# Tencent/PocketFlow

Measured on AMD Instinct MI355X. Metric: images/sec ResNet-50 INT8 quant-aware fine-tune (whole job; per GPU = value / n_gpus), higher is better.
Workload: dtype bf16

## Files before the change

pocketflow_amd/csrc/pf_api.hip:

```cpp
#include "pf_common.h"

extern "C" int pf_version(void) { return 100; }

extern "C" const char* pf_error_string(int err) {
  if (err == 0) return "ok";
  return hipGetErrorString((hipError_t)err);
}

#include <stdlib.h>
#include <stdio.h>
static PfTuning g_tuning;
static bool g_tuning_loaded = false;

static int env_int(const char* name, int dflt) {
  const char* e = getenv(name);
  return (e == nullptr || *e == 0) ? dflt : atoi(e);
}

static void tuning_load() {
  PfTuning t;
  t.conv_bn = env_int("PF_CONV_BN", 0);
  t.conv_igemm = env_int("PF_CONV_IGEMM", 1);
  t.conv_igemm_pro = env_int("PF_CONV_IGEMM_PRO", 1);
  t.conv_stream = env_int("PF_CONV_STREAM", 1);
  t.conv_stream_maxsplit = env_int("PF_CONV_STREAM_MAXSPLIT", 2);
  t.igemm_pro3 = env_int("PF_IGEMM_PRO3", 1);
  t.igemm_tile_bm = t.igemm_tile_bn = 0;
  const char* e = getenv("PF_IGEMM_TILE");
  if (e != nullptr) {
    int bm = 0, bn = 0;
    if (sscanf(e, "%dx%d", &bm, &bn) == 2) { t.igemm_tile_bm = bm; t.igemm_tile_bn = bn; }
  }
  t.pool3s2 = env_int("PF_POOL3S2", 1);
  t.wrw_tr = env_int("PF_WRW_TR", 0);
  t.wrw2 = env_int("PF_WRW2", 1);
  t.wrw2_target = env_int("PF_WRW2_TARGET", 0);
  t.splitk = env_int("PF_IGEMM_SPLITK", 1);
  t.wrw2_tk256 = env_int("PF_WRW2_TK256", 1);
  t.conv3x3_c64 = env_int("PF_CONV3X3_C64", 1);
  g_tuning = t;
  g_tuning_loaded = true;
}

const PfTuning& pf_tuning() {
  if (!g_tuning_loaded) tuning_load();
  return g_tuning;
}

extern "C" int pf_tuning_reload(void) { tuning_load(); return 0; }

#include <map>
#include <mutex>
#include <utility>
int pf_require_lds(const void* fn, size_t lds) {
  static std::mutex mu;
  static std::map<std::pair<int, const void*>, size_t> done;
  int dev = 0;
  hipError_t e = hipGetDevice(&dev);
  if (e != hipSuccess) return (int)e;
  std::lock_guard<std::mutex> lock(mu);
  size_t& have = done[std::make_pair(dev, fn)];
  if (lds > have) {
    e = hipFuncSetAttribute(fn, hipFuncAttributeMaxDynamicSharedMemorySize, (int)lds);
    if (e != hipSuccess) return (int)e;
    have = lds;
  }
  return 0;
}
```

pocketflow_amd/csrc/pf_common.h:

```cpp
#pragma once
#include <hip/hip_runtime.h>
#include <stdint.h>
#include "../../include/pocketflow_hip.h"

#define PF_WAVE 64
#define PF_THREADS 256
#define PF_MAX_GRID 2048

#define PF_LAUNCH_CHECK()                         \
  do {                                            \
    hipError_t e__ = hipGetLastError();           \
    if (e__ != hipSuccess) return (int)e__;       \
  } while (0)

typedef uint16_t bf16_t;

int pf_require_lds(const void* fn, size_t lds);

struct PfTuning {
  int conv_bn;
  int conv_igemm, conv_igemm_pro;
  int conv_stream;
  int conv_stream_maxsplit;
  int igemm_pro3;
  int igemm_tile_bm, igemm_tile_bn;
  int pool3s2;
  int wrw_tr, wrw2, wrw2_target;
  int wrw2_tk256;
  int splitk;
  int conv3x3_c64;
};
const PfTuning& pf_tuning();

__device__ __forceinline__ float bf16_to_f32(bf16_t h) {
  return __uint_as_float(((uint32_t)h) << 16);
}
__device__ __forceinline__ bf16_t f32_to_bf16(float f) {
  uint32_t u = __float_as_uint(f);
  if ((u & 0x7FFFFFFFu) > 0x7F800000u) return (bf16_t)((u >> 16) | 0x0040u);
  u += 0x7FFFu + ((u >> 16) & 1u);
  return (bf16_t)(u >> 16);
}

template <typename T> struct VecTraits;
template <> struct VecTraits<float> { static constexpr int N = 4; };
template <> struct VecTraits<bf16_t> { static constexpr int N = 8; };

template <typename T>
__device__ __forceinline__ void load_vec(const T* __restrict__ p, float* out);
template <>
__device__ __forceinline__ void load_vec<float>(const float* __restrict__ p, float* out) {
  float4 v = *reinterpret_cast<const float4*>(p);
  out[0] = v.x; out[1] = v.y; out[2] = v.z; out[3] = v.w;
}
template <>
__device__ __forceinline__ void load_vec<bf16_t>(const bf16_t* __restrict__ p, float* out) {
  uint4 v = *reinterpret_cast<const uint4*>(p);
  out[0] = __uint_as_float(v.x << 16); out[1] = __uint_as_float(v.x & 0xFFFF0000u);
  out[2] = __uint_as_float(v.y << 16); out[3] = __uint_as_float(v.y & 0xFFFF0000u);
  out[4] = __uint_as_float(v.z << 16); out[5] = __uint_as_float(v.z & 0xFFFF0000u);
  out[6] = __uint_as_float(v.w << 16); out[7] = __uint_as_float(v.w & 0xFFFF0000u);
}
template <typename T>
__device__ __forceinline__ void store_vec(T* __restrict__ p, const float* in);
template <>
__device__ __forceinline__ void store_vec<float>(float* __restrict__ p, const float* in) {
  *reinterpret_cast<float4*>(p) = make_float4(in[0], in[1], in[2], in[3]);
}
template <>
__device__ __forceinline__ void store_vec<bf16_t>(bf16_t* __restrict__ p, const float* in) {
  uint4 v;
  v.x = (uint32_t)f32_to_bf16(in[0]) | ((uint32_t)f32_to_bf16(in[1]) << 16);
  v.y = (uint32_t)f32_to_bf16(in[2]) | ((uint32_t)f32_to_bf16(in[3]) << 16);
  v.z = (uint32_t)f32_to_bf16(in[4]) | ((uint32_t)f32_to_bf16(in[5]) << 16);
  v.w = (uint32_t)f32_to_bf16(in[6]) | ((uint32_t)f32_to_bf16(in[7]) << 16);
  *reinterpret_cast<uint4*>(p) = v;
}
template <typename T> __device__ __forceinline__ void load8(const T* __restrict__ p, float* out);
template <> __device__ __forceinline__ void load8<float>(const float* __restrict__ p, float* out) {
  load_vec<float>(p, out); load_vec<float>(p + 4, out + 4);
}
template <> __device__ __forceinline__ void load8<bf16_t>(const bf16_t* __restrict__ p, float* out) {
  load_vec<bf16_t>(p, out);
}
template <typename T> __device__ __forceinline__ void store8(T* __restrict__ p, const float* in);
template <> __device__ __forceinline__ void store8<float>(float* __restrict__ p, const float* in) {
  store_vec<float>(p, in); store_vec<float>(p + 4, in + 4);
}
template <> __device__ __forceinline__ void store8<bf16_t>(bf16_t* __restrict__ p, const float* in) {
  store_vec<bf16_t>(p, in);
}
__host__ __device__ __forceinline__ bool pf_aligned16(const void* p) {
  return (((uintptr_t)p) & 15) == 0;
}
template <typename T> __device__ __forceinline__ float load_one(const T* p);
template <> __device__ __forceinline__ float load_one<float>(const float* p) { return *p; }
template <> __device__ __forceinline__ float load_one<bf16_t>(const bf16_t* p) { return bf16_to_f32(*p); }
template <typename T> __device__ __forceinline__ void store_one(T* p, float v);
template <> __device__ __forceinline__ void store_one<float>(float* p, float v) { *p = v; }
template <> __device__ __forceinline__ void store_one<bf16_t>(bf16_t* p, float v) { *p = f32_to_bf16(v); }

__device__ __forceinline__ uint32_t enc_f32(float f) {
  uint32_t u = __float_as_uint(f);
  return (u & 0x80000000u) ? ~u : (u | 0x80000000u);
}
__device__ __forceinline__ float dec_f32(uint32_t e) {
  uint32_t u = (e & 0x80000000u) ? (e & 0x7FFFFFFFu) : ~e;
  return __uint_as_float(u);
}
__device__ __forceinline__ void slot_alpha_beta(const uint32_t* slot, float& alpha, float& beta) {
  const uint2 sv = *reinterpret_cast<const uint2*>(slot);
// ... 71 lines not shown
```

pocketflow_amd/csrc/pf_conv.hip:

```cpp
#include "pf_conv_common.h"

template <int BN_T, bool PRO, bool BWD, bool MAP>
__global__ __launch_bounds__(PF_THREADS, 2) void k_conv1x1_fwd(const ConvArgs a) {
  constexpr int WM = (BN_T == 128) ? 64 : 32;
  constexpr int JM = WM / 16;
  constexpr int CS_LD = BN_T + 8;
  constexpr int VPR = BN_T / 8;
  constexpr int RPP = PF_THREADS / VPR;
  constexpr int NBV = BN_T * 8 / PF_THREADS;
  constexpr int A_EL = CV_BM * CV_LDK, B_EL = BN_T * CV_LDK;
  constexpr int C_EL = CV_BM * CS_LD;
  constexpr int RED_FL = 4 * RPP * BN_T;
  constexpr int SM_BYTES_AB = (A_EL + B_EL) * 2;
  constexpr int SM_BYTES = SM_BYTES_AB > RED_FL * 4 ? (SM_BYTES_AB > C_EL * 2 ? SM_BYTES_AB : C_EL * 2)
                                                    : RED_FL * 4;
  constexpr int SS_BYTES = PRO ? 2 * CV_MAXK * 4 : 0;
  __shared__ __attribute__((aligned(16))) unsigned char smem[SM_BYTES + SS_BYTES];
  float* ssl = reinterpret_cast<float*>(smem + SM_BYTES);
  __shared__ float bpl[BWD ? 4 * BN_T : 4];
  bf16_t* As = reinterpret_cast<bf16_t*>(smem);
  bf16_t* Bs = As + A_EL;
  bf16_t* Cs = reinterpret_cast<bf16_t*>(smem);
  float* red = reinterpret_cast<float*>(smem);

// ... 476 lines not shown
      if (vq[i]) v = *reinterpret_cast<const uint4*>(a.X + map_row(a, m) * a.K + k);
      rq[i] = v;
    }
  };
  auto sstore = [&]() {
#pragma unroll
    for (int i = 0; i < 4; ++i) {
      const int p = tid + i * PF_THREADS;
      st_transposed(Ds, (p & 15) * 8, p >> 4, rd[i]);
    }
#pragma unroll
    for (int i = 0; i < 2; ++i) {
      const int p = tid + i * PF_THREADS;
      uint4 v = rq[i];
      if (PRO) v = vq[i] ? pro_apply(pro, v) : make_uint4(0, 0, 0, 0);
      st_transposed(Qs, (p & 7) * 8, p >> 3, v);
    }
  };

  if (mbeg < mend) gload(mbeg);
  for (int mb = mbeg; mb < mend; mb += WR_BM) {
    sstore();
    __syncthreads();
    if (mb + WR_BM < mend) gload(mb + WR_BM);
#pragma unroll
    for (int kk = 0; kk < WR_BM / 32; ++kk) {
      bf16x8 df[2], qf[4];
      const int mg = kk * 4 + fm;
#pragma unroll
      for (int i = 0; i < 2; ++i) {
        const int c = wave * 32 + i * 16 + frow;
        df[i] = *reinterpret_cast<const bf16x8*>(Ds + c * WR_LDM + ((mg ^ ((c >> 3) & 7)) << 3));
      }
#pragma unroll
      for (int j = 0; j < 4; ++j) {
        const int c = j * 16 + frow;
        qf[j] = *reinterpret_cast<const bf16x8*>(Qs + c * WR_LDM + ((mg ^ ((c >> 3) & 7)) << 3));
      }
#pragma unroll
      for (int i = 0; i < 2; ++i)
#pragma unroll
        for (int j = 0; j < 4; ++j)
          acc[i][j] = __builtin_amdgcn_mfma_f32_16x16x32_bf16(df[i], qf[j], acc[i][j], 0, 0, 0);
    }
    __syncthreads();
  }
  float* out = a.partial + (int64_t)split * a.N * a.K;
#pragma unroll
  for (int i = 0; i < 2; ++i)
#pragma unroll
    for (int j = 0; j < 4; ++j) {
      const int k = k0 + j * 16 + (lane & 15);
#pragma unroll
      for (int r = 0; r < 4; ++r) {
        const int n = n0 + wave * 32 + i * 16 + (lane >> 4) * 4 + r;
        if (n < a.N && k < a.K) out[(int64_t)n * a.K + k] = acc[i][j][r];
      }
    }
}

template <typename TO>
__global__ __launch_bounds__(PF_THREADS) void k_wrw_reduce(const float* __restrict__ partial, int splits,
                                                           int64_t n, TO* __restrict__ out, int64_t out_stride) {
  __shared__ float l[4][64];
  const int e_l = threadIdx.x & 63, sg = threadIdx.x >> 6;
  const int64_t e = (int64_t)blockIdx.x * 64 + e_l;
  const int per = (splits + gridDim.y - 1) / gridDim.y;
  const int s0 = blockIdx.y * per, s1 = (s0 + per < splits) ? (s0 + per) : splits;
  float acc = 0.f;
  if (e < n)
    for (int s = s0 + sg; s < s1; s += 4) acc += partial[(int64_t)s * n + e];
  l[sg][e_l] = acc;
  __syncthreads();
  if (sg == 0 && e < n) store_one<TO>(out + (int64_t)blockIdx.y * out_stride + e, (l[0][e_l] + l[1][e_l]) + (l[2][e_l] + l[3][e_l]));
}

WrwPlan pf_wrw_plan(int M, int N, int C, int taps, bool entry_1x1, int64_t x_rows, int window_imgs);
int pf_wrw2_launch(const void* dY, const void* X, float* slabs, const float* scale_shift, int act, const uint32_t* slot,
                   int bits, int M, int N, int C, int th, int tw, int H, int Wd, int Ho, int Wo, int stride, int pad_h,
                   int pad_w, int S, int64_t x_rows, hipStream_t st);
int pf_wrw_tr_launch(const void* dY, const void* X, float* slabs, const float* scale_shift, int act,
                     const uint32_t* slot, int bits, int M, int N, int C, int th, int tw, int H, int Wd, int Ho, int Wo,
                     int stride, int pad_h, int pad_w, int S, hipStream_t st);

int pf_wrw_reduce(float* workspace, int S, int64_t n, void* dW, int dw_dtype, hipStream_t st) {
  const int gx = (int)((n + 63) / 64);
  int ry = 1;
  while (ry < 32 && gx * ry < 1024 && ry * 8 <= S) ry *= 2;
  float* stage = workspace + (int64_t)S * n;
  if (ry > 1) {
    k_wrw_reduce<float><<<dim3(gx, ry), PF_THREADS, 0, st>>>(workspace, S, n, stage, n);
    if (dw_dtype == PF_F32) k_wrw_reduce<float><<<dim3(gx, 1), PF_THREADS, 0, st>>>(stage, ry, n, (float*)dW, 0);
    else if (dw_dtype == PF_BF16) k_wrw_reduce<bf16_t><<<dim3(gx, 1), PF_THREADS, 0, st>>>(stage, ry, n, (bf16_t*)dW, 0);
    else return (int)hipErrorInvalidValue;
  } else {
    if (dw_dtype == PF_F32) k_wrw_reduce<float><<<dim3(gx, 1), PF_THREADS, 0, st>>>(workspace, S, n, (float*)dW, 0);
    else if (dw_dtype == PF_BF16) k_wrw_reduce<bf16_t><<<dim3(gx, 1), PF_THREADS, 0, st>>>(workspace, S, n, (bf16_t*)dW, 0);
    else return (int)hipErrorInvalidValue;
  }
  PF_LAUNCH_CHECK();
  return 0;
}

int pf_wrw_scatter_splits(int M, int N, int K) {
  const int tiles = ((N + WR_TN - 1) / WR_TN) * ((K + WR_TK - 1) / WR_TK);
  int S = (768 + tiles - 1) / tiles;
  const int maxS = (M + 4 * WR_BM - 1) / (4 * WR_BM);
  if (S > maxS) S = maxS;
  if (S < 1) S = 1;
  int rows = (M + S - 1) / S;
  rows = ((rows + WR_BM - 1) / WR_BM) * WR_BM;
  return (M + rows - 1) / rows;
}

extern "C" int pf_conv1x1_wrw_splits(int M, int N, int K) { return pf_wrw_plan(M, N, K, 1, true, 0, 0).S; }

extern "C" int pf_conv1x1_wrw(const void* dY, const void* X, void* dW, int dw_dtype, float* workspace,
                              const float* scale_shift, int act, const uint32_t* slot, int bits, int M, int N,
                              int K, int Ho, int Wo, int H, int Wd, int stride, void* stream) {
  if (M <= 0 || N <= 0 || K <= 0 || (K % 8) || (N % 8) || ((int64_t)N * K) % 4) return (int)hipErrorInvalidValue;
  if (!pf_aligned16(dY) || !pf_aligned16(X) || !pf_aligned16(workspace) || !pf_aligned16(dW))
    return (int)hipErrorInvalidValue;
  if (slot != nullptr && (bits < 1 || bits > 32 || scale_shift == nullptr)) return (int)hipErrorInvalidValue;
  if (stride < 1) stride = 1;
  hipStream_t st = (hipStream_t)stream;
  if (stride > 1 && (Ho <= 0 || Wo <= 0 || H <= 0 || Wd <= 0)) return (int)hipErrorInvalidValue;
  const int64_t x_rows = (stride > 1) ? (int64_t)(M / (Ho * Wo)) * H * Wd : (int64_t)M;
  const WrwPlan p = pf_wrw_plan(M, N, K, 1, true, x_rows, 0);
  int r = 0;
  if (p.kernel == WRW_SHARED) {
    r = pf_wrw2_launch(dY, X, workspace, scale_shift, act, slot, bits, M, N, K, 1, 1, H, Wd, Ho, Wo, stride, 0, 0, p.S, x_rows, st);
  } else if (p.kernel == WRW_WAVE) {
    r = pf_wrw_tr_launch(dY, X, workspace, scale_shift, act, slot, bits, M, N, K, 1, 1, H, Wd, Ho, Wo, stride, 0, 0, p.S, st);
  } else {
    ConvArgs a = conv_args(X, dY, nullptr, M, N, K);
    conv_args_prologue(a, scale_shift, act, slot, bits);
    conv_args_rowmap(a, Ho, Wo, H, Wd, stride, 0);
    a.partial = workspace;
    a.tiles_n = (N + WR_TN - 1) / WR_TN;
    const int tiles_k = (K + WR_TK - 1) / WR_TK;
    int rows = (M + p.S - 1) / p.S;
    rows = ((rows + WR_BM - 1) / WR_BM) * WR_BM;
    a.rows_per_split = rows;
    dim3 grid(a.tiles_n * tiles_k, p.S);
    if (scale_shift != nullptr) k_conv1x1_wrw<true><<<grid, PF_THREADS, 0, st>>>(a);
    else k_conv1x1_wrw<false><<<grid, PF_THREADS, 0, st>>>(a);
    PF_LAUNCH_CHECK();
  }
  if (r != 0) return r;
  return pf_wrw_reduce(workspace, p.S, (int64_t)N * K, dW, dw_dtype, st);
}
```

pocketflow_amd/csrc/pf_wrw.hip:

```cpp
#include "pf_conv_common.h"
#include <stdlib.h>

#define LDS_PTR(p) ((__attribute__((address_space(3))) void*)(p))
typedef short v4s __attribute__((ext_vector_type(4)));
typedef short v8s __attribute__((ext_vector_type(8)));

__device__ __attribute__((aligned(16))) const uint32_t pf_wrw_zero_page[64] = {0};

struct WrwArgs {
  const bf16_t* dY;
  const bf16_t* X;
  float* slabs;
  const float* ss;
  const uint32_t* slot;
  float kq, act_lo, act_hi;
  int M, N, C;
  int th, tw, H, Wd, Ho, Wo, stride, pad_h, pad_w;
  int tiles_n, tiles, rows_per_split;
};

template <int N> __device__ __forceinline__ void wrw_wait_vm() { asm volatile("s_waitcnt vmcnt(%0)" ::"n"(N) : "memory"); }

template <int BN, bool PRO, bool MAP>
__global__ __launch_bounds__(256) void k_wrw_tr(const WrwArgs a) {
  constexpr int NB = BN / 16;
  constexpr int NS = 3;
  constexpr int DY_BYTES = 4 * NB * 256, X_BYTES = 4 * 4 * 256, STAGE = DY_BYTES + X_BYTES;
  constexpr int LPS = NB + 4;
  constexpr int NBLK = NB * 4;
  extern __shared__ __attribute__((aligned(16))) unsigned char smem[];
  const int tid = threadIdx.x, lane = tid & 63;
  const int wave = __builtin_amdgcn_readfirstlane(tid >> 6);
  const int l15 = lane & 15, q = lane >> 4;
  unsigned char* ring = smem + wave * (NS * STAGE);
  const bf16_t* zero = reinterpret_cast<const bf16_t*>(pf_wrw_zero_page);

  const int nwg = gridDim.x;
  int wg = blockIdx.x;
  {
    const int xcd = wg & 7, idx = wg >> 3;
    const int qq = nwg >> 3, r = nwg & 7;
    wg = (xcd < r ? xcd * (qq + 1) : r * (qq + 1) + (xcd - r) * qq) + idx;
  }
  const int tile = wg % a.tiles, split = wg / a.tiles;
  const int tn = tile % a.tiles_n, tk = tile / a.tiles_n;
  const int n0 = tn * BN;
  const int cch = a.C >> 6;
  const int tap = tk / cch, c0 = (tk - tap * cch) * 64;
  const int tap_r = tap / a.tw, tap_s = tap - tap_r * a.tw;
  const int ktot = a.th * a.tw * a.C;
  const int mbeg = split * a.rows_per_split;
  const int mend = (mbeg + a.rows_per_split < a.M) ? (mbeg + a.rows_per_split) : a.M;
  const int nsteps = (mend > mbeg) ? (mend - mbeg + 31) / 32 : 0;
  const int my_steps = (nsteps > wave) ? (nsteps - wave + 3) / 4 : 0;

  float psc[4], psh[4];
  Pro pro;
  pro_init(pro, a.act_lo, a.act_hi, a.kq, PRO ? a.slot : nullptr);
  if (PRO) {
#pragma unroll
    for (int j = 0; j < 4; ++j) {
      psc[j] = pro_fold_scale(pro, a.ss[c0 + j * 16 + l15]);
      psh[j] = pro_fold_shift(pro, a.ss[a.C + c0 + j * 16 + l15]);
    }
  }

  const int sb = lane >> 4, srow = (lane & 15) >> 1, sch = lane & 1;
  const int hw_o = a.Ho * a.Wo;
  auto stage = [&](int step, int buf) {
    unsigned char* dst = ring + buf * STAGE;
    const int mb = mbeg + step * 32;
#pragma unroll
    for (int pg = 0; pg < 4; ++pg) {
      const int m = mb + pg * 8 + srow;
      const bool ok = m < mend;
#pragma unroll
      for (int g4 = 0; g4 < NB / 4; ++g4) {
        const int n = n0 + (g4 * 4 + sb) * 16 + sch * 8;
        const bf16_t* src = (ok && n < a.N) ? (a.dY + (int64_t)m * a.N + n) : (zero + sch * 8);
        __builtin_amdgcn_global_load_lds(src, LDS_PTR(dst + (pg * NB + g4 * 4) * 256), 16, 0, 0);
      }
      bool okx = ok;
      int64_t row = m;
      if (MAP && ok) {
// ... 162 lines not shown
#define PF_W_MAKE_RSRC(p, bytes) __builtin_amdgcn_make_buffer_rsrc((void*)(p), (short)0, (int)(bytes), 0x00020000)
#define PF_W_BUFFER_LOAD_LDS16(rs, lds, voff) __builtin_amdgcn_raw_ptr_buffer_load_lds(rs, LDS_PTR(lds), 16, voff, 0, 0, 0)
#else
typedef int pf_wrsrc_t;
#define PF_W_MAKE_RSRC(p, bytes) 0
#define PF_W_BUFFER_LOAD_LDS16(rs, lds, voff) ((void)(rs), (void)(lds), (void)(voff))
#endif

#ifndef PF_W2_ABLATE
#define PF_W2_ABLATE 0
#endif
#ifdef PF_W2_TIMING
#define PF_W2_STAMP(k) do { if (blockIdx.x == (unsigned)tm_blk && t >= 4 && t < 12 && lane == 0) \
    tm_out[(t - 4) * 8 + (k)] = (uint32_t)__builtin_readcyclecounter(); } while (0)
#else
#define PF_W2_STAMP(k) do { } while (0)
#endif

__device__ __forceinline__ bf16x8 tr_join(const v4s& lo, const v4s& hi) {
  v8s x8;
  x8[0] = lo[0]; x8[1] = lo[1]; x8[2] = lo[2]; x8[3] = lo[3];
  x8[4] = hi[0]; x8[5] = hi[1]; x8[6] = hi[2]; x8[7] = hi[3];
  return *reinterpret_cast<const bf16x8*>(&x8);
}
template <int HI>
__device__ __forceinline__ void tr_read_frags(uint32_t p, bf16x8 (&f)[4]) {
  v4s l0, l1, l2, l3, h0, h1, h2, h3;
  asm volatile("ds_read_b64_tr_b16 %0, %8\n\tds_read_b64_tr_b16 %4, %8 offset:%9\n\t"
               "ds_read_b64_tr_b16 %1, %8 offset:256\n\tds_read_b64_tr_b16 %5, %8 offset:%10\n\t"
               "ds_read_b64_tr_b16 %2, %8 offset:512\n\tds_read_b64_tr_b16 %6, %8 offset:%11\n\t"
               "ds_read_b64_tr_b16 %3, %8 offset:768\n\tds_read_b64_tr_b16 %7, %8 offset:%12\n\t"
               "s_waitcnt lgkmcnt(0)"
               : "=&v"(l0), "=&v"(l1), "=&v"(l2), "=&v"(l3), "=&v"(h0), "=&v"(h1), "=&v"(h2), "=&v"(h3)
               : "v"(p), "n"(HI), "n"(HI + 256), "n"(HI + 512), "n"(HI + 768)
               : "memory");
  f[0] = tr_join(l0, h0); f[1] = tr_join(l1, h1); f[2] = tr_join(l2, h2); f[3] = tr_join(l3, h3);
}
template <int HI>
__device__ __forceinline__ void tr_read_frags(uint32_t p, bf16x8 (&f)[2]) {
  v4s l0, l1, h0, h1;
  asm volatile("ds_read_b64_tr_b16 %0, %4\n\tds_read_b64_tr_b16 %2, %4 offset:%5\n\t"
               "ds_read_b64_tr_b16 %1, %4 offset:256\n\tds_read_b64_tr_b16 %3, %4 offset:%6\n\t"
               "s_waitcnt lgkmcnt(0)"
               : "=&v"(l0), "=&v"(l1), "=&v"(h0), "=&v"(h1)
               : "v"(p), "n"(HI), "n"(HI + 256)
               : "memory");
  f[0] = tr_join(l0, h0); f[1] = tr_join(l1, h1);
}

template <int HIX, int HID>
__device__ __forceinline__ void tr_read_frags2(uint32_t px, uint32_t pd, bf16x8 (&xf)[4], bf16x8 (&df)[4]) {
  v4s a0, a1, a2, a3, b0, b1, b2, b3, c0, c1, c2, c3, d0, d1, d2, d3;
  asm volatile("ds_read_b64_tr_b16 %0, %16\n\tds_read_b64_tr_b16 %4, %16 offset:%18\n\t"
               "ds_read_b64_tr_b16 %1, %16 offset:256\n\tds_read_b64_tr_b16 %5, %16 offset:%19\n\t"
               "ds_read_b64_tr_b16 %2, %16 offset:512\n\tds_read_b64_tr_b16 %6, %16 offset:%20\n\t"
               "ds_read_b64_tr_b16 %3, %16 offset:768\n\tds_read_b64_tr_b16 %7, %16 offset:%21\n\t"
               "ds_read_b64_tr_b16 %8, %17\n\tds_read_b64_tr_b16 %12, %17 offset:%22\n\t"
               "ds_read_b64_tr_b16 %9, %17 offset:256\n\tds_read_b64_tr_b16 %13, %17 offset:%23\n\t"
               "ds_read_b64_tr_b16 %10, %17 offset:512\n\tds_read_b64_tr_b16 %14, %17 offset:%24\n\t"
               "ds_read_b64_tr_b16 %11, %17 offset:768\n\tds_read_b64_tr_b16 %15, %17 offset:%25\n\t"
               "s_waitcnt lgkmcnt(0)"
               : "=&v"(a0), "=&v"(a1), "=&v"(a2), "=&v"(a3), "=&v"(b0), "=&v"(b1), "=&v"(b2), "=&v"(b3),
                 "=&v"(c0), "=&v"(c1), "=&v"(c2), "=&v"(c3), "=&v"(d0), "=&v"(d1), "=&v"(d2), "=&v"(d3)
               : "v"(px), "v"(pd), "n"(HIX), "n"(HIX + 256), "n"(HIX + 512), "n"(HIX + 768), "n"(HID), "n"(HID + 256), "n"(HID + 512),
                 "n"(HID + 768)
               : "memory");
  xf[0] = tr_join(a0, b0); xf[1] = tr_join(a1, b1); xf[2] = tr_join(a2, b2); xf[3] = tr_join(a3, b3);
  df[0] = tr_join(c0, d0); df[1] = tr_join(c1, d1); df[2] = tr_join(c2, d2); df[3] = tr_join(c3, d3);
}

struct Wrw2Args {
  const bf16_t* dY;
  const bf16_t* X;
  float* slabs;
  const float* ss;
  const uint32_t* slot;
  float kq, act_lo, act_hi;
  uint32_t dy_bytes, x_bytes;
  int M, N, C;
  int th, tw, H, Wd, Ho, Wo, stride, pad_h, pad_w;
  int tiles_n, tiles, rows_per_split;
};

template <int TN, int TK, int WTN, int WTK, bool PRO, int MAPM>
__global__ __launch_bounds__(64 * (TN / WTN) * (TK / WTK)) void k_wrw2(const Wrw2Args a) {
  constexpr int WN = TN / WTN, WK = TK / WTK, NWAVE = WN * WK;
  constexpr int NI = WTN / 16, NJ = WTK / 16;
  constexpr int NBN = TN / 16, NBK = TK / 16;
  constexpr int DY_BYTES = 4 * NBN * 256, X_BYTES = 4 * NBK * 256, STAGE = DY_BYTES + X_BYTES;
  constexpr int IDY = 4 * (TN / 64), IX = 4 * (TK / 64);
  static_assert(IDY % NWAVE == 0 || IDY < NWAVE, "dY instructions must split evenly over the wavefronts (slot kinds are static)");
  constexpr int KDY = (IDY + NWAVE - 1) / NWAVE;
  constexpr int XS = (IX + NWAVE - 1) / NWAVE;
  extern __shared__ __attribute__((aligned(16))) unsigned char smem[];
  const int tid = threadIdx.x, lane = tid & 63;
  const int wave = __builtin_amdgcn_readfirstlane(tid >> 6);
  const int l15 = lane & 15, q = lane >> 4;
  const int wn = wave / WK, wk = wave % WK;

  const int nwg = gridDim.x;
  int wg = blockIdx.x;
  {
    const int xcd = wg & 7, idx = wg >> 3;
    const int qq = nwg >> 3, r = nwg & 7;
    wg = (xcd < r ? xcd * (qq + 1) : r * (qq + 1) + (xcd - r) * qq) + idx;
  }
  const int tile = wg % a.tiles, split = wg / a.tiles;
  const int tn = tile % a.tiles_n, tk = tile / a.tiles_n;
  const int n0 = tn * TN;
  const int kt = a.C / TK;
  const int tap = tk / kt, c0 = (tk - tap * kt) * TK;
  const int tap_r = tap / a.tw, tap_s = tap - tap_r * a.tw;
  const int ktot = a.th * a.tw * a.C;
  const int mbeg = split * a.rows_per_split;
  const int mend = (mbeg + a.rows_per_split < a.M) ? (mbeg + a.rows_per_split) : a.M;
  const int nsteps = (mend > mbeg) ? (mend - mbeg + 31) / 32 : 0;

  const pf_wrsrc_t rsY = PF_W_MAKE_RSRC(a.dY, (uint32_t)mend * (uint32_t)a.N * 2u);
  const pf_wrsrc_t rsX = PF_W_MAKE_RSRC(a.X, (MAPM == 0) ? (uint32_t)mend * (uint32_t)a.C * 2u : a.x_bytes);
  constexpr uint32_t OOB = 0x80000000u;
  const int sb = lane >> 4, srow = (lane & 15) >> 1, sch = lane & 1;
  const int hw_o = a.Ho * a.Wo;

  float psc[XS][8], psh[XS][8];
  Pro pro;
  pro_init(pro, a.act_lo, a.act_hi, a.kq, PRO ? a.slot : nullptr);
  if (PRO) {
#pragma unroll
    for (int x = 0; x < XS; ++x) {
      const int xi = wave + x * NWAVE;
      if (xi < IX) {
        const int g4 = xi % (TK / 64);
        const int c = c0 + (g4 * 4 + sb) * 16 + sch * 8;
#pragma unroll
        for (int j = 0; j < 8; ++j) { psc[x][j] = pro_fold_scale(pro, a.ss[c + j]); psh[x][j] = pro_fold_shift(pro, a.ss[a.C + c + j]); }
      }
    }
  }

  uint32_t yoff[KDY], xoff[XS];
  const uint32_t ystep = 32u * (uint32_t)a.N * 2u, xstep = 32u * (uint32_t)a.C * 2u;
#pragma unroll
  for (int k = 0; k < KDY; ++k) {
    const int id = (wave + k * NWAVE) % IDY;
    const int pg = id / (TN / 64), g4 = id % (TN / 64);
    const int n = n0 + (g4 * 4 + sb) * 16 + sch * 8;
    yoff[k] = (n < a.N && wave + k * NWAVE < IDY) ? (uint32_t)((mbeg + pg * 8 + srow) * a.N + n) * 2u : OOB;
  }
  int px_img[XS], px_ho[XS], px_wo[XS];
  const int adv_q = 32 / a.Wo, adv_r = 32 - adv_q * a.Wo;
  const int tap_dr = tap_r - a.pad_h, tap_ds = tap_s - a.pad_w;
#pragma unroll
  for (int x = 0; x < XS; ++x) {
    const int xi = (wave + x * NWAVE) % IX;
    const int pg = xi / (TK / 64), g4 = xi % (TK / 64);
    const int m = mbeg + pg * 8 + srow;
    const int cofs = c0 + (g4 * 4 + sb) * 16 + sch * 8;
    px_img[x] = 0; px_ho[x] = 0; px_wo[x] = 0;
    if (MAPM != 0) {
      const int img = m / hw_o, rem = m - img * hw_o;
      px_img[x] = img; px_ho[x] = rem / a.Wo; px_wo[x] = rem - px_ho[x] * a.Wo;
    }
    const int row0 = (MAPM == 1) ? m + tap_dr * a.Wd + tap_ds : m;
    xoff[x] = (uint32_t)(row0 * a.C + cofs) * 2u;
  }
  auto stage = [&](int step, int buf) {
    unsigned char* dst = smem + buf * STAGE;
// ... 36 lines not shown
      }
      if (!own) voff = OOB;
      unsigned char* xdst = own ? dst + DY_BYTES + (pg * NBK + g4 * 4) * 256 : smem + 3 * STAGE;
      if (!(PF_W2_ABLATE & 2)) PF_W_BUFFER_LOAD_LDS16(rsX, xdst, voff);
    }
  };
  auto transform = [&](int buf) {
    unsigned char* dst = smem + buf * STAGE;
#pragma unroll
    for (int x = 0; x < XS; ++x) {
      const int xi = wave + x * NWAVE;
      if (xi < IX) {
        const int pg = xi / (TK / 64), g4 = xi % (TK / 64);
#pragma unroll
        for (int j = 0; j < 8; ++j) { pro.sc[j] = psc[x][j]; pro.sh[j] = psh[x][j]; }
        const uint32_t p = lds_addr(dst + DY_BYTES + (pg * NBK + g4 * 4) * 256 + lane * 16);
        lds_write_b128(p, pro_apply(pro, lds_read_b128(p)));
      }
    }
  };

  f32x4 acc[NI][NJ];
#pragma unroll
  for (int i = 0; i < NI; ++i)
#pragma unroll
    for (int j = 0; j < NJ; ++j) acc[i][j] = (f32x4){0.f, 0.f, 0.f, 0.f};
  const int tr_off = (q & 1) * 128 + (l15 >> 2) * 32 + (l15 & 3) * 8;
  const int pg_lo = q >> 1;

  constexpr int NSTG = 3, LPS = KDY + XS;
  if (nsteps > 0) stage(0, 0);
  if (nsteps > 1) { stage(1, 1); wrw_wait_vm<LPS>(); } else wrw_wait_vm<0>();
  if (PRO && nsteps > 0) transform(0);
  asm volatile("s_waitcnt lgkmcnt(0)" ::: "memory");
  __builtin_amdgcn_s_barrier();
  int buf = 0, ibuf = 2;
#ifdef PF_W2_TIMING
  const int tm_blk = gridDim.x / 2;
  uint32_t* tm_out = reinterpret_cast<uint32_t*>(a.slabs) + wave * 64;
#endif
  for (int t = 0; t < nsteps; ++t) {
    const bool more2 = t + 2 < nsteps;
    PF_W2_STAMP(0);
    if (more2) { stage(t + 2, ibuf); ibuf = (ibuf + 1 == NSTG) ? 0 : ibuf + 1; }
    PF_W2_STAMP(1);
    const unsigned char* sbase = smem + buf * STAGE;
    buf = (buf + 1 == NSTG) ? 0 : buf + 1;
    if (!(PF_W2_ABLATE & 1)) {
      bf16x8 xf[NJ], df[NI];
      if constexpr (NI == 4 && NJ == 4) {
        tr_read_frags2<2 * NBK * 256, 2 * NBN * 256>(lds_addr(sbase + DY_BYTES + (pg_lo * NBK + wk * NJ) * 256 + tr_off),
                                                     lds_addr(sbase + (pg_lo * NBN + wn * NI) * 256 + tr_off), xf, df);
      } else
      {
      tr_read_frags<2 * NBK * 256>(lds_addr(sbase + DY_BYTES + (pg_lo * NBK + wk * NJ) * 256 + tr_off), xf);
      tr_read_frags<2 * NBN * 256>(lds_addr(sbase + (pg_lo * NBN + wn * NI) * 256 + tr_off), df);
      }
      PF_W2_STAMP(2);
#pragma unroll
      for (int i = 0; i < NI; ++i)
#pragma unroll
        for (int j = 0; j < NJ; ++j)
          acc[i][j] = __builtin_amdgcn_mfma_f32_16x16x32_bf16(df[i], xf[j], acc[i][j], 0, 0, 0);
    }
    __builtin_amdgcn_sched_barrier(0);
    PF_W2_STAMP(3);
    if (t + 1 < nsteps) {
      if (more2) wrw_wait_vm<LPS>(); else wrw_wait_vm<0>();
      PF_W2_STAMP(4);
      if (PRO) transform(buf);
    }
    asm volatile("s_waitcnt lgkmcnt(0)" ::: "memory");
    PF_W2_STAMP(5);
    __builtin_amdgcn_s_barrier();
    __builtin_amdgcn_sched_barrier(0);
    PF_W2_STAMP(6);
  }
#ifdef PF_W2_TIMING
  return;
#endif

  float* out = a.slabs + (int64_t)split * a.N * ktot;
  const int kcol = tap * a.C + c0 + wk * WTK;
#pragma unroll
  for (int i = 0; i < NI; ++i)
#pragma unroll
    for (int j = 0; j < NJ; ++j) {
      const int k = kcol + j * 16 + l15;
      const int n = n0 + wn * WTN + i * 16 + q * 4;
#pragma unroll
      for (int r = 0; r < 4; ++r)
        if (n + r < a.N && (!(PF_W2_ABLATE & 4) || acc[i][j][r] == 12345.678f)) out[(int64_t)(n + r) * ktot + k] = acc[i][j][r];
    }
}

struct Wrw2Cfg { int tn, tk; };
static Wrw2Cfg wrw2_pick(int N, int C) {
  const int tn = (N % 256 == 0) ? 256 : ((N % 128 == 0) ? 128 : 64);
  int tk = (C % 128 == 0) ? 128 : 64;
  if (tn <= 128 && C % 256 == 0 && pf_tuning().wrw2_tk256 != 0) tk = 256;
  if (tn == 128 && tk == 64) return Wrw2Cfg{64, 64};
  return Wrw2Cfg{tn, tk};
}

static bool wrw2_fits(int M, int N, int C, int64_t x_rows) {
  return (int64_t)M * N < ((int64_t)1 << 30) && x_rows * C < ((int64_t)1 << 30);
}

int pf_wrw2_splits(int M, int N, int C, int taps) {
  if (pf_tuning().wrw2 == 0) return 0;
  if ((C % 64) || (N % 64) || M < 2048 || !wrw2_fits(M, N, C, 0)) return 0;
  const Wrw2Cfg c = wrw2_pick(N, C);
  const int tiles = (N / c.tn) * (taps * C / c.tk);
  const int forced = pf_tuning().wrw2_target;
  const int target = (forced > 0) ? forced : (taps == 1 ? 256 : 384);
  int S = (target + tiles - 1) / tiles;
  const int maxS = (M + 255) / 256;
  if (S > maxS) S = maxS;
  if (S < 1) S = 1;
  int rows = (M + S - 1) / S;
  rows = ((rows + 31) / 32) * 32;
  return (M + rows - 1) / rows;
}

template <int TN, int TK, int WTN, int WTK, bool PRO, int MAPM>
static int wrw2_launch_t(const Wrw2Args& a, int grid, hipStream_t st) {
  const size_t lds = 3 * (size_t)(4 * (TN / 16) * 256 + 4 * (TK / 16) * 256) + 1024;
  if (int e = pf_require_lds(reinterpret_cast<const void*>(&k_wrw2<TN, TK, WTN, WTK, PRO, MAPM>), lds)) return e;
  k_wrw2<TN, TK, WTN, WTK, PRO, MAPM><<<grid, 64 * (TN / WTN) * (TK / WTK), lds, st>>>(a);
  PF_LAUNCH_CHECK();
  return 0;
}

int pf_wrw2_launch(const void* dY, const void* X, float* slabs, const float* scale_shift, int act, const uint32_t* slot,
                   int bits, int M, int N, int C, int th, int tw, int H, int Wd, int Ho, int Wo, int stride, int pad_h,
                   int pad_w, int S, int64_t x_rows, hipStream_t st) {
  if (S <= 0 || !wrw2_fits(M, N, C, x_rows)) return (int)hipErrorInvalidValue;
  Wrw2Args a;
  a.dY = (const bf16_t*)dY; a.X = (const bf16_t*)X; a.slabs = slabs; a.ss = scale_shift; a.slot = slot;
  a.kq = uq_k_of_bits(slot ? bits : 8);
  pf_act_window(act, &a.act_lo, &a.act_hi);
  a.dy_bytes = (uint32_t)((int64_t)M * N * 2);
  a.x_bytes = (uint32_t)(x_rows * C * 2);
  a.M = M; a.N = N; a.C = C; a.th = th; a.tw = tw; a.H = H; a.Wd = Wd; a.Ho = Ho; a.Wo = Wo;
  a.stride = stride; a.pad_h = pad_h; a.pad_w = pad_w;
  const Wrw2Cfg c = wrw2_pick(N, C);
  a.tiles_n = N / c.tn;
  a.tiles = a.tiles_n * (th * tw * C / c.tk);
  int rows = (M + S - 1) / S;
  rows = ((rows + 31) / 32) * 32;
  a.rows_per_split = rows;
  const int grid = a.tiles * S;
  const bool pro = scale_shift != nullptr;
  int mapm = 0;
  if (stride != 1 || th * tw > 1) mapm = (stride == 1 && Ho == H && Wo == Wd && 32 / Wo + 1 <= Ho) ? 1 : 2;
  if (pro && th * tw > 1) return (int)hipErrorInvalidValue;
  if (pro && mapm == 1) mapm = 2;
#define PF_W2(TNV, TKV, WTNV, WTKV)                                                                           \
  do {                                                                                                        \
    if (pro) return mapm ? wrw2_launch_t<TNV, TKV, WTNV, WTKV, true, 2>(a, grid, st)                           \
                         : wrw2_launch_t<TNV, TKV, WTNV, WTKV, true, 0>(a, grid, st);                          \
    if (mapm == 1) return wrw2_launch_t<TNV, TKV, WTNV, WTKV, false, 1>(a, grid, st);                          \
    return mapm ? wrw2_launch_t<TNV, TKV, WTNV, WTKV, false, 2>(a, grid, st)                                   \
                : wrw2_launch_t<TNV, TKV, WTNV, WTKV, false, 0>(a, grid, st);                                  \
  } while (0)
  if (c.tn == 128 && c.tk == 256) PF_W2(128, 256, 64, 64);
  if (c.tn == 64 && c.tk == 256) PF_W2(64, 256, 32, 64);
  if (c.tn == 256 && c.tk == 128) PF_W2(256, 128, 64, 64);
  if (c.tn == 128 && c.tk == 128) PF_W2(128, 128, 64, 64);
  if (c.tn == 256 && c.tk == 64) PF_W2(256, 64, 64, 32);
  if (c.tn == 64 && c.tk == 128) PF_W2(64, 128, 32, 64);
  PF_W2(64, 64, 32, 32);
#undef PF_W2
}

int pf_wrw_reduce(float* workspace, int S, int64_t n, void* dW, int dw_dtype, hipStream_t st);

bool pf_wrw3x3_c64_geom(int H, int Wd, int C, int N, int th, int tw, int stride, int pad_h, int pad_w, int Ho, int Wo);
bool pf_wrw3x3_c64_fits(int imgs);
int pf_wrw3x3_c64_splits(int imgs);
int pf_wrw3x3_c64_launch(const void* dY, const void* X, float* slabs, int imgs, hipStream_t st);
int pf_wrw_scatter_splits(int M, int N, int K);

WrwPlan pf_wrw_plan(int M, int N, int C, int taps, bool entry_1x1, int64_t x_rows, int window_imgs) {
  if (window_imgs > 0 && pf_wrw3x3_c64_fits(window_imgs)) return WrwPlan{WRW_WINDOW, pf_wrw3x3_c64_splits(window_imgs)};
  const int s2 = pf_wrw2_splits(M, N, C, taps);
  if (s2 > 0) return WrwPlan{wrw2_fits(M, N, C, x_rows) ? WRW_SHARED : WRW_WAVE, s2};
  const int s1 = (!entry_1x1 || pf_tuning().wrw_tr != 0) ? wrw_tr_splits(M, N, C, taps) : 0;
  if (s1 > 0) return WrwPlan{WRW_WAVE, s1};
  if (entry_1x1) return WrwPlan{WRW_SCATTER, pf_wrw_scatter_splits(M, N, C)};
  return WrwPlan{WRW_NONE, 0};
}

extern "C" int pf_conv2d_wrw_splits(int M, int N, int C, int taps) {
  const int s = pf_wrw_plan(M, N, C, taps, false, 0, 0).S;
  if (pf_tuning().conv3x3_c64 != 0 && taps == 9 && N == 64 && C == 64 && M % (56 * 56) == 0) {
    const int s3 = pf_wrw_plan(M, N, C, taps, false, 0, M / (56 * 56)).S;
    return s3 > s ? s3 : s;
  }
  return s;
}

extern "C" int pf_conv2d_wrw(const void* dY, const void* X, void* dW, int dw_dtype, float* workspace, int imgs, int H,
                             int Wd, int C, int N, int th, int tw, int stride, int pad_h, int pad_w, int Ho, int Wo,
                             void* stream) {
  if (imgs <= 0 || H <= 0 || Wd <= 0 || Ho <= 0 || Wo <= 0 || th < 1 || tw < 1 || stride < 1) return (int)hipErrorInvalidValue;
  if (!pf_aligned16(dY) || !pf_aligned16(X) || !pf_aligned16(dW) || !pf_aligned16(workspace)) return (int)hipErrorInvalidValue;
  const int M = imgs * Ho * Wo;
  hipStream_t st = (hipStream_t)stream;
  const bool window = pf_wrw3x3_c64_geom(H, Wd, C, N, th, tw, stride, pad_h, pad_w, Ho, Wo);
  const WrwPlan p = pf_wrw_plan(M, N, C, th * tw, false, (int64_t)imgs * H * Wd, window ? imgs : 0);
  int r = (int)hipErrorInvalidValue;
  if (p.kernel == WRW_WINDOW) r = pf_wrw3x3_c64_launch(dY, X, workspace, imgs, st);
  if (p.kernel == WRW_SHARED)
    r = pf_wrw2_launch(dY, X, workspace, nullptr, PF_ACT_NONE, nullptr, 8, M, N, C, th, tw, H, Wd, Ho, Wo, stride, pad_h, pad_w, p.S,
                       (int64_t)imgs * H * Wd, st);
  if (p.kernel == WRW_WAVE)
    r = pf_wrw_tr_launch(dY, X, workspace, nullptr, PF_ACT_NONE, nullptr, 8, M, N, C, th, tw, H, Wd, Ho, Wo, stride, pad_h, pad_w, p.S, st);
  if (r != 0) return r;
  return pf_wrw_reduce(workspace, p.S, (int64_t)N * th * tw * C, dW, dw_dtype, st);
}
```

Measured before the change: 11410.

## Store wrw2 partials in MFMA fragment layout and add matching fragment-aware reduce

The weight-gradient wrw2 kernel now writes each accumulator fragment as one contiguous float4 per lane in a 16x16-blocked layout instead of a row-major scatter, which makes the partial-slab stores coalesced. A new two-stage reduce kernel sums the split slabs in that blocked layout, optionally staging through extra workspace, and transposes back to row-major dW in the final pass. This is on by default through PF_WRW2_FRAG. It adds constraints that N and ktot be multiples of 16, needs extra workspace for the staging pass, and may add a launch.

```diff
diff --git a/pocketflow_amd/csrc/pf_api.hip b/pocketflow_amd/csrc/pf_api.hip
--- a/pocketflow_amd/csrc/pf_api.hip
+++ b/pocketflow_amd/csrc/pf_api.hip
@@ -37,6 +37,7 @@
   t.wrw2_target = env_int("PF_WRW2_TARGET", 0);
   t.splitk = env_int("PF_IGEMM_SPLITK", 1);
   t.wrw2_tk256 = env_int("PF_WRW2_TK256", 1);
+  t.wrw2_frag = env_int("PF_WRW2_FRAG", 1);
   t.conv3x3_c64 = env_int("PF_CONV3X3_C64", 1);
   g_tuning = t;
   g_tuning_loaded = true;
diff --git a/pocketflow_amd/csrc/pf_common.h b/pocketflow_amd/csrc/pf_common.h
--- a/pocketflow_amd/csrc/pf_common.h
+++ b/pocketflow_amd/csrc/pf_common.h
@@ -27,6 +27,7 @@
   int pool3s2;
   int wrw_tr, wrw2, wrw2_target;
   int wrw2_tk256;
+  int wrw2_frag;
   int splitk;
   int conv3x3_c64;
 };
diff --git a/pocketflow_amd/csrc/pf_conv.hip b/pocketflow_amd/csrc/pf_conv.hip
--- a/pocketflow_amd/csrc/pf_conv.hip
+++ b/pocketflow_amd/csrc/pf_conv.hip
@@ -582,6 +582,7 @@
 int pf_wrw_tr_launch(const void* dY, const void* X, float* slabs, const float* scale_shift, int act,
                      const uint32_t* slot, int bits, int M, int N, int C, int th, int tw, int H, int Wd, int Ho, int Wo,
                      int stride, int pad_h, int pad_w, int S, hipStream_t st);
+int pf_wrw2_reduce(float* workspace, int S, int N, int ktot, void* dW, int dw_dtype, hipStream_t st);
 
 int pf_wrw_reduce(float* workspace, int S, int64_t n, void* dW, int dw_dtype, hipStream_t st) {
   const int gx = (int)((n + 63) / 64);
@@ -648,5 +649,6 @@
     PF_LAUNCH_CHECK();
   }
   if (r != 0) return r;
+  if (p.kernel == WRW_SHARED) return pf_wrw2_reduce(workspace, p.S, N, K, dW, dw_dtype, st);
   return pf_wrw_reduce(workspace, p.S, (int64_t)N * K, dW, dw_dtype, st);
 }
diff --git a/pocketflow_amd/csrc/pf_wrw.hip b/pocketflow_amd/csrc/pf_wrw.hip
--- a/pocketflow_amd/csrc/pf_wrw.hip
+++ b/pocketflow_amd/csrc/pf_wrw.hip
@@ -1,5 +1,6 @@
 #include "pf_conv_common.h"
 #include <stdlib.h>
+#include <type_traits>
 
 #define LDS_PTR(p) ((__attribute__((address_space(3))) void*)(p))
 typedef short v4s __attribute__((ext_vector_type(4)));
@@ -328,7 +329,7 @@
   int tiles_n, tiles, rows_per_split;
 };
 
-template <int TN, int TK, int WTN, int WTK, bool PRO, int MAPM>
+template <int TN, int TK, int WTN, int WTK, bool PRO, int MAPM, bool FRAG>
 __global__ __launch_bounds__(64 * (TN / WTN) * (TK / WTK)) void k_wrw2(const Wrw2Args a) {
   constexpr int WN = TN / WTN, WK = TK / WTK, NWAVE = WN * WK;
   constexpr int NI = WTN / 16, NJ = WTK / 16;
@@ -531,6 +532,17 @@
 
   float* out = a.slabs + (int64_t)split * a.N * ktot;
   const int kcol = tap * a.C + c0 + wk * WTK;
+  if constexpr (FRAG) {
+    float4* out4 = reinterpret_cast<float4*>(out) + ((int64_t)((n0 + wn * WTN) >> 4) * (ktot >> 4) + (kcol >> 4)) * 64 + lane;
+    const int64_t nb_stride = (int64_t)(ktot >> 4) * 64;
+#pragma unroll
+    for (int i = 0; i < NI; ++i)
+#pragma unroll
+      for (int j = 0; j < NJ; ++j)
+        if (!(PF_W2_ABLATE & 4) || acc[i][j][0] == 12345.678f)
+          out4[i * nb_stride + j * 64] = make_float4(acc[i][j][0], acc[i][j][1], acc[i][j][2], acc[i][j][3]);
+    return;
+  }
 #pragma unroll
   for (int i = 0; i < NI; ++i)
 #pragma unroll
@@ -572,20 +584,28 @@
   return (M + rows - 1) / rows;
 }
 
-template <int TN, int TK, int WTN, int WTK, bool PRO, int MAPM>
-static int wrw2_launch_t(const Wrw2Args& a, int grid, hipStream_t st) {
+template <int TN, int TK, int WTN, int WTK, bool PRO, int MAPM, bool FRAG>
+static int wrw2_launch_f(const Wrw2Args& a, int grid, hipStream_t st) {
   const size_t lds = 3 * (size_t)(4 * (TN / 16) * 256 + 4 * (TK / 16) * 256) + 1024;
-  if (int e = pf_require_lds(reinterpret_cast<const void*>(&k_wrw2<TN, TK, WTN, WTK, PRO, MAPM>), lds)) return e;
-  k_wrw2<TN, TK, WTN, WTK, PRO, MAPM><<<grid, 64 * (TN / WTN) * (TK / WTK), lds, st>>>(a);
+  if (int e = pf_require_lds(reinterpret_cast<const void*>(&k_wrw2<TN, TK, WTN, WTK, PRO, MAPM, FRAG>), lds)) return e;
+  k_wrw2<TN, TK, WTN, WTK, PRO, MAPM, FRAG><<<grid, 64 * (TN / WTN) * (TK / WTK), lds, st>>>(a);
   PF_LAUNCH_CHECK();
   return 0;
+}
+
+template <int TN, int TK, int WTN, int WTK, bool PRO, int MAPM>
+static int wrw2_launch_t(const Wrw2Args& a, bool frag, int grid, hipStream_t st) {
+  if (frag) return wrw2_launch_f<TN, TK, WTN, WTK, PRO, MAPM, true>(a, grid, st);
+  return wrw2_launch_f<TN, TK, WTN, WTK, PRO, MAPM, false>(a, grid, st);
 }
 
 int pf_wrw2_launch(const void* dY, const void* X, float* slabs, const float* scale_shift, int act, const uint32_t* slot,
                    int bits, int M, int N, int C, int th, int tw, int H, int Wd, int Ho, int Wo, int stride, int pad_h,
                    int pad_w, int S, int64_t x_rows, hipStream_t st) {
   if (S <= 0 || !wrw2_fits(M, N, C, x_rows)) return (int)hipErrorInvalidValue;
+  if ((N % 16) || ((th * tw * C) % 16)) return (int)hipErrorInvalidValue;
   Wrw2Args a;
+  const bool frag = pf_tuning().wrw2_frag != 0;
   a.dY = (const bf16_t*)dY; a.X = (const bf16_t*)X; a.slabs = slabs; a.ss = scale_shift; a.slot = slot;
   a.kq = uq_k_of_bits(slot ? bits : 8);
   pf_act_window(act, &a.act_lo, &a.act_hi);
@@ -605,13 +625,13 @@
   if (stride != 1 || th * tw > 1) mapm = (stride == 1 && Ho == H && Wo == Wd && 32 / Wo + 1 <= Ho) ? 1 : 2;
   if (pro && th * tw > 1) return (int)hipErrorInvalidValue;
   if (pro && mapm == 1) mapm = 2;
-#define PF_W2(TNV, TKV, WTNV, WTKV)                                                                           \
-  do {                                                                                                        \
-    if (pro) return mapm ? wrw2_launch_t<TNV, TKV, WTNV, WTKV, true, 2>(a, grid, st)                           \
-                         : wrw2_launch_t<TNV, TKV, WTNV, WTKV, true, 0>(a, grid, st);                          \
-    if (mapm == 1) return wrw2_launch_t<TNV, TKV, WTNV, WTKV, false, 1>(a, grid, st);                          \
-    return mapm ? wrw2_launch_t<TNV, TKV, WTNV, WTKV, false, 2>(a, grid, st)                                   \
-                : wrw2_launch_t<TNV, TKV, WTNV, WTKV, false, 0>(a, grid, st);                                  \
+#define PF_W2(TNV, TKV, WTNV, WTKV)                                                                                   \
+  do {                                                                                                                \
+    if (pro) return mapm ? wrw2_launch_t<TNV, TKV, WTNV, WTKV, true, 2>(a, frag, grid, st)                            \
+                         : wrw2_launch_t<TNV, TKV, WTNV, WTKV, true, 0>(a, frag, grid, st);                           \
+    if (mapm == 1) return wrw2_launch_t<TNV, TKV, WTNV, WTKV, false, 1>(a, frag, grid, st);                           \
+    return mapm ? wrw2_launch_t<TNV, TKV, WTNV, WTKV, false, 2>(a, frag, grid, st)                                    \
+                : wrw2_launch_t<TNV, TKV, WTNV, WTKV, false, 0>(a, frag, grid, st);                                   \
   } while (0)
   if (c.tn == 128 && c.tk == 256) PF_W2(128, 256, 64, 64);
   if (c.tn == 64 && c.tk == 256) PF_W2(64, 256, 32, 64);
@@ -623,7 +643,71 @@
 #undef PF_W2
 }
 
+template <typename TO, bool FINAL>
+__global__ __launch_bounds__(PF_THREADS) void k_wrw2_reduce(const float4* __restrict__ partial, int splits, int64_t n4,
+                                                            TO* __restrict__ out, int64_t out_stride, int kblocks, int ktot) {
+  __shared__ float4 l[4][64];
+  const int lane = threadIdx.x & 63, sg = __builtin_amdgcn_readfirstlane(threadIdx.x >> 6);
+  const int per = (splits + gridDim.y - 1) / gridDim.y;
+  const int s0 = blockIdx.y * per, s1 = (s0 + per < splits) ? (s0 + per) : splits;
+  const int64_t step = 4 * n4;
+  const float4* p = partial + (int64_t)blockIdx.x * 64 + lane + (int64_t)(s0 + sg) * n4;
+  float4 acc = make_float4(0.f, 0.f, 0.f, 0.f);
+  auto fold = [&](auto u_tag) {
+    constexpr int U = decltype(u_tag)::value;
+    float4 v[U];
+#pragma unroll
+    for (int u = 0; u < U; ++u) v[u] = p[u * step];
+#pragma unroll
+    for (int u = 0; u < U; ++u) { acc.x += v[u].x; acc.y += v[u].y; acc.z += v[u].z; acc.w += v[u].w; }
+    p += U * step;
+  };
+  int left = (s1 - s0 - sg + 3) >> 2;
+  for (; left >= 8; left -= 8) fold(std::integral_constant<int, 8>());
+  if (left >= 4) { fold(std::integral_constant<int, 4>()); left -= 4; }
+  if (left == 3) fold(std::integral_constant<int, 3>());
+  else if (left == 2) fold(std::integral_constant<int, 2>());
+  else if (left == 1) fold(std::integral_constant<int, 1>());
+  l[sg][lane] = acc;
+  __syncthreads();
+  if (FINAL) {
+    const int row = threadIdx.x >> 4, col = threadIdx.x & 15;
+    const int src = (row >> 2) * 16 + col, r = row & 3;
+    const float* lf = reinterpret_cast<const float*>(&l[0][0]);
+    const float v = (lf[(0 * 64 + src) * 4 + r] + lf[(1 * 64 + src) * 4 + r]) + (lf[(2 * 64 + src) * 4 + r] + lf[(3 * 64 + src) * 4 + r]);
+    const int nb = blockIdx.x / kblocks, kb = blockIdx.x - nb * kblocks;
+    store_one<TO>(out + (int64_t)(nb * 16 + row) * ktot + kb * 16 + col, v);
+  } else if (sg == 0) {
+    const float4 a = l[0][lane], b = l[1][lane], c = l[2][lane], d = l[3][lane];
+    reinterpret_cast<float4*>(out)[(int64_t)blockIdx.y * out_stride + (int64_t)blockIdx.x * 64 + lane] =
+        make_float4((a.x + b.x) + (c.x + d.x), (a.y + b.y) + (c.y + d.y), (a.z + b.z) + (c.z + d.z), (a.w + b.w) + (c.w + d.w));
+  }
+}
+
 int pf_wrw_reduce(float* workspace, int S, int64_t n, void* dW, int dw_dtype, hipStream_t st);
+
+int pf_wrw2_reduce(float* workspace, int S, int N, int ktot, void* dW, int dw_dtype, hipStream_t st) {
+  const int64_t n = (int64_t)N * ktot;
+  if (pf_tuning().wrw2_frag == 0) return pf_wrw_reduce(workspace, S, n, dW, dw_dtype, st);
+  if ((N % 16) || (ktot % 16) || (dw_dtype != PF_F32 && dw_dtype != PF_BF16)) return (int)hipErrorInvalidValue;
+  const int gx = (int)((n + 63) / 64);
+  int ry = 1;
+  while (ry < 32 && gx * ry < 1024 && ry * 8 <= S) ry *= 2;
+  const int blocks = (int)(n / 256), kblocks = ktot / 16;
+  const float4* slabs = reinterpret_cast<const float4*>(workspace);
+  int splits = S;
+  if (ry > 1) {
+    float* stage = workspace + (int64_t)S * n;
+    k_wrw2_reduce<float, false><<<dim3(blocks, ry), PF_THREADS, 0, st>>>(slabs, S, n / 4, stage, n / 4, kblocks, ktot);
+    slabs = reinterpret_cast<const float4*>(stage);
+    splits = ry;
+  }
+  if (dw_dtype == PF_F32) k_wrw2_reduce<float, true><<<dim3(blocks, 1), PF_THREADS, 0, st>>>(slabs, splits, n / 4, (float*)dW, 0, kblocks, ktot);
+  else k_wrw2_reduce<bf16_t, true><<<dim3(blocks, 1), PF_THREADS, 0, st>>>(slabs, splits, n / 4, (bf16_t*)dW, 0, kblocks, ktot);
+  PF_LAUNCH_CHECK();
+  return 0;
+}
+
 
 bool pf_wrw3x3_c64_geom(int H, int Wd, int C, int N, int th, int tw, int stride, int pad_h, int pad_w, int Ho, int Wo);
 bool pf_wrw3x3_c64_fits(int imgs);
@@ -667,5 +751,6 @@
   if (p.kernel == WRW_WAVE)
     r = pf_wrw_tr_launch(dY, X, workspace, nullptr, PF_ACT_NONE, nullptr, 8, M, N, C, th, tw, H, Wd, Ho, Wo, stride, pad_h, pad_w, p.S, st);
   if (r != 0) return r;
+  if (p.kernel == WRW_SHARED) return pf_wrw2_reduce(workspace, p.S, N, th * tw * C, dW, dw_dtype, st);
   return pf_wrw_reduce(workspace, p.S, (int64_t)N * th * tw * C, dW, dw_dtype, st);
 }
```

Measured after the change: 11410. About the same (-0.0%).
